# cristian-jfv/lattice-boltzmann-method

Hardware: AMD Instinct MI355X
Metric: MLUPS (million lattice updates/sec), D2Q9 BGK periodic box, f64 (higher is better)
Workload: dtype f64

## Files before the change

lattice-boltzmann-method_amd/csrc/capi_kbc.hip:

```cpp
#include "kbc.hpp"
#include "launch.hpp"

namespace lbm {

__global__ __launch_bounds__(256) void k_kbc_equilibrium(double* __restrict__ feq,
                                                         const double* __restrict__ m0,
                                                         const double* __restrict__ m1, long n,
                                                         int zero_u2) {
  for (long i = (long)blockIdx.x * 256 + threadIdx.x; i < n; i += (long)gridDim.x * 256) {
    const double ux = m1[i], uy = m1[n + i];
    const double ux2 = zero_u2 ? 0.0 : ux * ux, uy2 = zero_u2 ? 0.0 : uy * uy;
    double e[Q];
    KbcModel::feq_poly(e, ux, uy, ux2, uy2);
    const double r = m0[i];
#pragma unroll
    for (int q = 0; q < Q; ++q) feq[q * n + i] = e[q] * r;
  }
}

__global__ __launch_bounds__(256) void k_kbc_collide_given(double* __restrict__ out,
                                                           const double* __restrict__ f,
                                                           const double* __restrict__ m0,
                                                           const double* __restrict__ m1, long n,
                                                           KbcModel m) {
// ... 75 lines not shown
static int launch_stream_collide_sw_kbc(const char* fn, double* pn, const double* po,
                                        const lbm_geom* lg, const lbm_bc* lbc, const KbcFastModel& m,
                                        int depth, int row_begin, int row_end, hipStream_t st) {
  SwArgs a;
  int rc = sw_check_args(fn, pn, po, lg, lbc, depth, row_begin, row_end, sw_full_strips<KbcFastModel>::value, kSwKbc, &a);
  if (rc || !a.nrows) return rc;
  if (a.walls) {
    rc = depth == 2 ? sw_launch_walls<KbcFastModel, 2>(pn, po, a.g, m, a.bc, row_begin, row_end, st)
                    : sw_launch_walls<KbcFastModel, 3>(pn, po, a.g, m, a.bc, row_begin, row_end, st);
    if (rc) return rc;
    LBM_CHECK_LAUNCH();
    return LBM_OK;
  }
  auto launch = [&](auto D, auto LDSR) {
    constexpr int DV = decltype(D)::value;
    const SwPlan p = sw_plan(k_stream_collide_sw<KbcFastModel, DV, 2, true, false, false, LDSR()>, 128, a.nrows, a.strips, depth);
    LBM_KLAUNCH((k_stream_collide_sw<KbcFastModel, DV, 2, true, false, false, LDSR()>), dim3((p.n_waves + 1) / 2), dim3(128), 0, st, pn, po, a.g, m,
                row_begin, row_end, p.rpc, a.strips, p.n_waves, tuning("sw_xcd", 0));
  };
  with_flags([&](auto LDSR) {
    switch (depth) {
      case 2: launch(std::integral_constant<int, 2>{}, LDSR); break;
      case 3: launch(std::integral_constant<int, 3>{}, LDSR); break;
      default: launch(std::integral_constant<int, 4>{}, LDSR); break;
    }
  }, tuning("sw_ldsring", 1) != 0);
  LBM_CHECK_LAUNCH();
  return LBM_OK;
}

}
int lbm::kbc_stream_collide_x2_ref(double* pn, const double* po, const lbm_geom* lg, const lbm_bc* lbc,
                                   const lbm_kbc_params* prm, int row_begin, int row_end, hipStream_t st) {
// ... 126 lines not shown
```

lattice-boltzmann-method_amd/csrc/d2q9.hpp:

```cpp
#pragma once
#include <type_traits>
#include <hip/hip_runtime.h>

#include "../../include/lbm_hip.h"

namespace lbm {

constexpr int Q = 9;

#define LBM_W0 (4.0 / 9.0)
#define LBM_WS (1.0 / 9.0)
#define LBM_WD (1.0 / 36.0)

__device__ __forceinline__ constexpr double wq(int q) {
  return q == 0 ? LBM_W0 : (q < 5 ? LBM_WS : LBM_WD);
}
__host__ __device__ __forceinline__ constexpr int icx(int q) {
  return (q == 1 || q == 5 || q == 8) ? 1 : ((q == 3 || q == 6 || q == 7) ? -1 : 0);
}
__host__ __device__ __forceinline__ constexpr int icy(int q) {
  return (q == 2 || q == 5 || q == 6) ? 1 : ((q == 4 || q == 7 || q == 8) ? -1 : 0);
}
__host__ __device__ __forceinline__ constexpr int opp(int q) {
  return q == 0 ? 0 : (q == 1 ? 3 : (q == 2 ? 4 : (q == 3 ? 1 : (q == 4 ? 2 : (q == 5 ? 7 : (q == 6 ? 8 : (q == 7 ? 5 : 6)))))));
// ... 603 lines not shown
  (void)c_load;
}

#ifdef LBM_EXPERIMENTS
#include "experiments/sw_prefetch2.hpp"
#endif

__host__ __device__ constexpr int sw_strip_width(int D, bool full = false) {
  return full ? 64 - 2 * (D - 1) : (64 - 2 * (D - 1)) / 8 * 8;
}
template <class M, class = void>
struct sw_full_strips : std::false_type {};
template <class M>
struct sw_full_strips<M, std::void_t<decltype(M::kFullStrips)>> : std::bool_constant<M::kFullStrips> {};
__host__ __device__ constexpr int sw_waves_per_simd(int D) { return D <= 2 ? 4 : (D == 3 ? 3 : (D <= 5 ? 2 : 1)); }
template <class Model, int D, bool NT_STORE, bool HAS_BC, bool PF2, bool LDSR = false>
__device__ __forceinline__ void sw_wave_body(double* __restrict__ pn, const double* __restrict__ po, const Geom& g,
                                             const Model& m, int row_begin, int row_end, int rows_per_chunk, int strips,
                                             int wave, int lane, const Bc& bc, int strip0, int chunk_stride,
                                             double* lds = nullptr) {
  static_assert(!(LDSR && (HAS_BC || PF2)), "the LDS ring exists for the plain window only");
  constexpr int W = sw_strip_width(D, sw_full_strips<Model>::value);
  const int strip = strip0 + wave % strips, chunk = wave / strips;
  const int R0 = row_begin + chunk * (chunk_stride > 0 ? chunk_stride : rows_per_chunk);
  const int R1 = R0 + rows_per_chunk < row_end ? R0 + rows_per_chunk : row_end;
  int c = strip * W - (D - 1) + lane;
  const int c_raw = c;
  const bool lane_ok = lane >= D - 1 && lane < D - 1 + W && c < g.C;
  const bool walled_cols = HAS_BC && (bc_is_wall(bc.col_lo) || bc_is_wall(bc.col_hi));
  if (walled_cols) {
    c = c < 0 ? 0 : (c > g.C - 1 ? g.C - 1 : c);
  } else {
    c = c < 0 ? c + g.C : (c >= g.C ? c - g.C : c);
    c = c >= g.C ? c - g.C : c;
  }
  const int cols[3] = {walled_cols ? (c + 1 > g.C - 1 ? g.C - 1 : c + 1) : wrap_col(g, c + 1), c,
                       walled_cols ? (c - 1 < 0 ? 0 : c - 1) : wrap_col(g, c - 1)};
  const int rbase = R0 - (D - 1);
  const int n_iter = (R1 - R0) + 2 * (D - 1);
  double ring[D > 1 ? D - 1 : 1][3][Q];
// ... 44 lines not shown
  if constexpr (LDSR) {
    for (int k = lane; k < sw_lds_ring_doubles(D); k += 64) lds[k] = 1.0;
    __builtin_amdgcn_fence(__ATOMIC_RELEASE, "wavefront");
    __builtin_amdgcn_wave_barrier();
    __builtin_amdgcn_fence(__ATOMIC_ACQUIRE, "wavefront");
  }
  for (int i = 0; i < n_iter; i += 3) {
    sw_iteration<Model, D, 0, NT_STORE, HAS_BC, LDSR>(ring, cur, pn, po, g, m, i, rbase, R0, R1, c, cols, lane_ok, c, bc, c_bc, lds, lane);
    sw_iteration<Model, D, 1, NT_STORE, HAS_BC, LDSR>(ring, cur, pn, po, g, m, i + 1, rbase, R0, R1, c, cols, lane_ok, c, bc, c_bc, lds, lane);
    sw_iteration<Model, D, 2, NT_STORE, HAS_BC, LDSR>(ring, cur, pn, po, g, m, i + 2, rbase, R0, R1, c, cols, lane_ok, c, bc, c_bc, lds, lane);
  }
}

template <class Model, int D, int WAVES, bool NT_STORE, bool HAS_BC = false, bool PF2 = false, bool LDSR = false>
__global__ __launch_bounds__(64 * WAVES, (LDSR ? 2 : (WAVES == 4 ? sw_waves_per_simd(D) : 1))) void k_stream_collide_sw(
    double* __restrict__ pn, const double* __restrict__ po, Geom g, Model m, int row_begin,
    int row_end, int rows_per_chunk, int strips, int n_waves, int xcd_group, Bc bc = Bc{}, int strip0 = 0,
    int chunk_stride = 0) {
  int blk = blockIdx.x;
  if (xcd_group > 0) {
    const int x = blk % 8, mth = blk / 8, win = 8 * xcd_group;
    if ((mth / xcd_group + 1) * win <= (int)gridDim.x) blk = (mth / xcd_group) * win + x * xcd_group + mth % xcd_group;
  }
  const int wave = blk * WAVES + __builtin_amdgcn_readfirstlane(threadIdx.x >> 6), lane = threadIdx.x & 63;
  if (wave >= n_waves) return;
  if constexpr (LDSR) {
    __shared__ double lring[WAVES * sw_lds_ring_doubles(D)];
    sw_wave_body<Model, D, NT_STORE, HAS_BC, PF2, true>(pn, po, g, m, row_begin, row_end, rows_per_chunk, strips, wave, lane, bc, strip0, chunk_stride,
                                                        lring + (threadIdx.x >> 6) * sw_lds_ring_doubles(D));
  } else {
    sw_wave_body<Model, D, NT_STORE, HAS_BC, PF2>(pn, po, g, m, row_begin, row_end, rows_per_chunk, strips, wave, lane, bc, strip0, chunk_stride);
  }
}

struct SwPart {
  int r0, r1, s0, ns, rpc, wave0;
};
struct SwParts {
  SwPart p[5];
  int n_frame_waves, n_waves;
};
template <class Model, int D, bool NT_STORE>
__global__ __launch_bounds__(128, 1) void k_stream_collide_sw_walls(double* __restrict__ pn, const double* __restrict__ po,
                                                                    Geom g, Model m, Bc bc, SwParts parts) {
  const int wave = blockIdx.x * 2 + __builtin_amdgcn_readfirstlane(threadIdx.x >> 6), lane = threadIdx.x & 63;
  if (wave >= parts.n_waves) return;
  if (wave < parts.n_frame_waves) {
    int k = 0;
#pragma unroll
    for (int a = 1; a < 4; ++a)
      if (parts.p[a].ns > 0 && parts.p[a].r1 > parts.p[a].r0 && wave >= parts.p[a].wave0) k = a;
    const SwPart pt = parts.p[k];
    sw_wave_body<Model, D, NT_STORE, true, false>(pn, po, g, m, pt.r0, pt.r1, pt.rpc, pt.ns, wave - pt.wave0, lane, bc, pt.s0, 0);
  } else {
    const SwPart pt = parts.p[4];
    sw_wave_body<Model, D, NT_STORE, false, false>(pn, po, g, m, pt.r0, pt.r1, pt.rpc, pt.ns, wave - pt.wave0, lane, bc, pt.s0, 0);
  }
}

#ifdef LBM_EXPERIMENTS
#include "experiments/sw_paired_strips.hpp"
#endif
#ifdef LBM_EXPERIMENTS
#include "experiments/sw_two_columns.hpp"
#endif

template <class Model, bool WITH_MOMENTS>
__global__ __launch_bounds__(256) void k_edge_stream_collide(
    double* __restrict__ pn, const double* __restrict__ po, Geom g, Bc bc, Model m, int row_begin,
    int row_end, double* __restrict__ rho_out, double* __restrict__ u_out) {
  const int i = blockIdx.x * blockDim.x + threadIdx.x, n = row_end - row_begin;
// ... 52 lines not shown
```

lattice-boltzmann-method_amd/csrc/experiments/cg_launch.hpp:

```cpp
constexpr bool kCgExperiments = true;
constexpr int kCgNotMine = 1;

template <class Kernel>
static SwPlan cg_exp_chunks(Kernel* kernel, int block_threads, int nrows, int strips, int depth = 3, int rows_unfitted = 64) {
  return sw_plan(kernel, block_threads, nrows, strips, depth, 0, "cg_rows2", rows_unfitted);
}

template <int WAVES>
static int launch_cg_strip_t(const CgStepArgs& a, hipStream_t st) {
  int rpc = tuning("cg_rows", 16);
  const int nrows = a.row_end - a.row_begin;
  if (rpc > nrows) rpc = nrows;
  const int strips = (a.g.C + CG_SW - 1) / CG_SW, chunks = (nrows + rpc - 1) / rpc;
  const int n_waves = strips * chunks;
  const dim3 grid((n_waves + WAVES - 1) / WAVES);
  with_flags([&](auto PSI) { LBM_KLAUNCH((k_cg_strip<WAVES, PSI()>), grid, dim3(64 * WAVES), 0, st, a.pn_r, a.pn_b, a.in_r, a.in_b, a.g, a.bc, a.cf, a.rho_r, a.rho_b, a.u, a.psi, a.snu, a.mi, a.row_begin, a.row_end, rpc, strips, n_waves); }, a.psi != nullptr);
  LBM_CHECK_LAUNCH();
  return LBM_OK;
}

template <int TR, int TC, int WAVES>
static int cg_exp_one_launch(const CgStepArgs& a, const CgPlan& p, int part, int xs, hipStream_t st) {
  switch (a.g.P != a.g.C ? 0 : tuning("cg_strip", 0)) {
    case 0: break;
// ... 13 lines not shown
  with_flags([&](auto PSI) { LBM_KLAUNCH((k_cg_tile_mn<BR, BC, BT, BM, BP, PSI()>), dim3(p.n_btr * p.n_btc), dim3(BT), 0, st, a.pn_r, a.pn_b, a.in_r, a.in_b, a.g, a.cf, a.rho_r, a.rho_b, a.u, a.psi, a.snu, a.mi, ra, ca, p.n_btc, p.big_xcd); }, a.psi != nullptr);
}

static void cg_exp_walk_tile(const CgStepArgs& a, const CgPlan& p, int ra, int ca, hipStream_t st) {
  int rpc = tuning("cg_walk_rows", 128) / 16 * 16;
  if (rpc < 16) rpc = 16;
  const int rows_total = p.n_btr * 16, chunks = (rows_total + rpc - 1) / rpc;
  const int wx = tuning("cg_walk_tile_xcd", 2);
  with_flags([&](auto PSI) { LBM_KLAUNCH((k_cg_walk_tile<PSI()>), dim3(chunks * p.n_btc), dim3(512), 0, st, a.pn_r, a.pn_b, a.in_r, a.in_b, a.g, a.cf, a.rho_r, a.rho_b, a.u, a.psi, a.snu, a.mi, ra, ca, p.n_btc, rows_total, rpc, wx); }, a.psi != nullptr);
}

template <int WV>
static void cg_exp_strip2(const CgStepArgs& a, int ra, int rb, int ca, int cb, hipStream_t st) {
  const int strips = (cb - ca + CG_SW2 - 1) / CG_SW2;
  with_flags([&](auto PSI) {
    const SwPlan c = cg_exp_chunks(k_cg_strip2<WV, PSI()>, 64 * WV, rb - ra, strips);
    LBM_KLAUNCH((k_cg_strip2<WV, PSI()>), dim3((c.n_waves + WV - 1) / WV), dim3(64 * WV), 0, st, a.pn_r, a.pn_b, a.in_r, a.in_b, a.g, a.cf, a.rho_r, a.rho_b, a.u, a.psi, a.snu, a.mi, ra, rb, ca, cb, c.rpc, strips, c.n_waves);
  }, a.psi != nullptr);
}

template <int WV>
static void cg_exp_strip3(const CgStepArgs& a, int ra, int rb, int ca, int cb, hipStream_t st) {
  const int strips = (cb - ca + CG_SW2 - 1) / CG_SW2;
  const int xo = tuning("cg_strip_xcd", 0);
  with_flags([&](auto PSI) {
    const SwPlan c = cg_exp_chunks(k_cg_strip3<WV, PSI()>, 64 * WV, rb - ra, strips);
    const int nblk = (c.n_waves + WV - 1) / WV, grid = xo ? ((nblk + 7) / 8) * 8 : nblk;
    LBM_KLAUNCH((k_cg_strip3<WV, PSI()>), dim3(grid), dim3(64 * WV), 0, st, a.pn_r, a.pn_b, a.in_r, a.in_b, a.g, a.cf, a.rho_r, a.rho_b, a.u, a.psi, a.snu, a.mi, ra, rb, ca, cb, c.rpc, strips, c.n_waves, xo);
  }, a.psi != nullptr);
}

template <int WV>
static void cg_exp_strip4(const CgStepArgs& a, int ra, int rb, int ca, int cb, hipStream_t st) {
  constexpr int S = 64 * WV - 2 * CG_S4_EDGE;
  const int win0 = (ca - CG_S4_EDGE) / 16 * 16;
  const int bstrips = (cb - (win0 + CG_S4_EDGE) + S - 1) / S;
  with_flags([&](auto PSI) {
    const int rpc = cg_exp_chunks(k_cg_strip4<WV, PSI()>, 64 * WV, rb - ra, bstrips * WV).rpc;
    const int chunks = (rb - ra + rpc - 1) / rpc;
    LBM_KLAUNCH((k_cg_strip4<WV, PSI()>), dim3(bstrips * chunks), dim3(64 * WV), 0, st, a.pn_r, a.pn_b, a.in_r, a.in_b, a.g, a.cf, a.rho_r, a.rho_b, a.u, a.psi, a.snu, a.mi, ra, rb, ca, cb, rpc, bstrips, win0);
  }, a.psi != nullptr);
// ... 143 lines not shown
```

lattice-boltzmann-method_amd/csrc/launch.hpp:

```cpp
#pragma once
#include <map>
#include <mutex>
#include <utility>
#include "d2q9.hpp"
#include "internal.hpp"

namespace lbm {

inline int validate_geom_bc(const char* fn, const lbm_geom* g, const lbm_bc* bc, bool reads_neighbours = true) {
  LBM_REQUIRE(g, "%s: NULL geometry", fn);
  LBM_REQUIRE(g->R >= 1 && g->C >= 1, "%s: R=%d C=%d must be positive", fn, g->R, g->C);
  LBM_REQUIRE(g->ghost >= 0 && g->ghost <= 15, "%s: ghost=%d must be 0..15", fn, g->ghost);
  LBM_REQUIRE(g->row_pitch == 0 || (g->row_pitch >= g->C && g->row_pitch % 2 == 0), "%s: row_pitch=%d must be even and >= C=%d (0 = dense)",
              fn, g->row_pitch, g->C);
  LBM_REQUIRE(g->plane_stride == 0 || g->plane_stride >= (long long)(g->R + 2 * g->ghost) * (g->row_pitch > 0 ? g->row_pitch : g->C),
              "%s: plane_stride=%lld smaller than a plane", fn, g->plane_stride);
  if (bc) {
    auto row_ok = [](int m) {
      return m == LBM_EDGE_PERIODIC || m == LBM_EDGE_HALO || m == LBM_EDGE_BOUNCE_BACK ||
             m == LBM_EDGE_ABB_VELOCITY;
    };
    auto col_ok = [](int m) {
      return m == LBM_EDGE_PERIODIC || m == LBM_EDGE_BOUNCE_BACK || m == LBM_EDGE_SPECULAR ||
             m == LBM_EDGE_WRAP_NOSHIFT;
// ... 117 lines not shown
    with_flags([&](auto NS) {                                                                     \
      LBM_KLAUNCH((k_stream_collide_tb2<Model, TRV, BV, NS()>), dim3((unsigned)nblk), dim3(BV), 0, st, pn, po, g, m, \
                  row_begin, row_end, tiles_x, tiles_y, order);                                   \
    }, nt);                                                                                       \
  } else
  LBM_TB2(4, 256) LBM_TB2(6, 256) LBM_TB2(8, 256) LBM_TB2(8, 512) LBM_TB2(12, 256) LBM_TB2(12, 512)
  LBM_TB2(14, 512) LBM_TB2(16, 512) LBM_TB2(16, 1024) LBM_TB2(30, 1024) {
    set_error("%s: no two-step instantiation for tb_rows=%d tb_block=%d", fn, tr, block);
    return LBM_ERR_INVALID;
  }
#undef LBM_TB2
  LBM_CHECK_LAUNCH();
  return LBM_OK;
}

inline int sw_pick_rows(int nrows, int strips, int depth, long slots) {
  auto cost = [&](int rows) {
    const long waves = (long)strips * ((nrows + rows - 1) / rows);
    const long rounds = (waves + slots - 1) / slots;
    return (double)rounds * (rows + 2 * (depth - 1)) * (1.0 + 0.25 / ((double)rounds * (double)rounds));
  };
  int best = nrows < 64 ? nrows : 64;
  double best_cost = cost(best) * 0.95;
  for (int rows = 32; rows <= 256 && rows <= nrows; rows += 4) {
    const double c = cost(rows);
    if (c < best_cost) best = rows, best_cost = c;
  }
  return best;
}

inline long sw_wave_slots(const void* kernel, int block_threads) {
  static std::mutex mu;
  static std::map<std::pair<const void*, int>, long> cache;
  int dev = 0;
  if (hipGetDevice(&dev) != hipSuccess) {
    (void)hipGetLastError();
    return 0;
  }
  std::lock_guard<std::mutex> lk(mu);
  auto it = cache.find({kernel, dev});
  if (it != cache.end()) return it->second;
  int blocks_per_cu = 0, cus = 0;
  long slots = 0;
  if (hipOccupancyMaxActiveBlocksPerMultiprocessor(&blocks_per_cu, kernel, block_threads, 0) == hipSuccess &&
      hipDeviceGetAttribute(&cus, hipDeviceAttributeMultiprocessorCount, dev) == hipSuccess && blocks_per_cu > 0 && cus > 0)
    slots = (long)blocks_per_cu * (block_threads / 64) * cus;
  else
    (void)hipGetLastError();
  cache[{kernel, dev}] = slots;
  return slots;
}

struct SwPlan {
  int rpc, n_waves;
};
template <class Kernel>
SwPlan sw_plan(Kernel* kernel, int block_threads, int nrows, int strips, int depth, int rows_fixed = 0,
               const char* rows_key = "sw_rows", int rows_unfitted = 64) {
  int rpc = rows_fixed > 0 ? rows_fixed : tuning(rows_key, -1);
  if (rpc <= 0) {
    const long slots = sw_wave_slots((const void*)kernel, block_threads);
    rpc = slots > 0 ? sw_pick_rows(nrows, strips, depth, slots) : rows_unfitted;
  }
  if (rpc > nrows) rpc = nrows;
  return {rpc, strips * ((nrows + rpc - 1) / rpc)};
}

template <class Model, int DV, bool HAS_BC>
void sw_launch_part(double* pn, const double* po, const Geom& g, const Model& m, const Bc& bc, int r0,
                    int r1, int s0, int ns, int rows_fixed, hipStream_t st) {
  if (r0 >= r1 || ns <= 0) return;
  const SwPlan p = sw_plan(k_stream_collide_sw<Model, DV, 2, true, HAS_BC>, 128, r1 - r0, ns, DV, rows_fixed);
  LBM_KLAUNCH((k_stream_collide_sw<Model, DV, 2, true, HAS_BC>), dim3((p.n_waves + 1) / 2), dim3(128), 0, st, pn, po, g, m,
              r0, r1, p.rpc, ns, p.n_waves, 0, bc, s0);
}

struct SwSideStream : SideStream {
  int dev = -1;
};
inline SideStream* sw_side_stream() {
  static thread_local SwSideStream side[16];
  int dev = 0;
  if (hipGetDevice(&dev) != hipSuccess || dev < 0 || dev >= 16) return nullptr;
  SwSideStream& s = side[dev];
  if (s.dev != dev) {
    if (s.create()) {
      (void)hipGetLastError();
      return nullptr;
    }
// ... 13 lines not shown
  if (bc_is_wall(bc.row_hi)) rb = row_end < g.R - 16 ? row_end : g.R - 16;
  if (col_walls) {
    s0 = 1;
    s1 = (g.C - W - DV) / W + 1;
    if (s1 > strips) s1 = strips;
  }
  int split = tuning("sw_split", -1);
  if (split < 0) split = (row_begin == 0 && row_end == g.R && !g.ghost) ? 1 : 2;
  if (split == 0 || ra >= rb || s0 >= s1) {
    sw_launch_part<Model, DV, true>(pn, po, g, m, bc, row_begin, row_end, 0, strips, 0, st);
    return LBM_OK;
  }
  if (split == 2) {
    SwParts pp{};
    const int fr = 8;
    auto part = [&](int k, int r0, int r1, int s0f, int ns, int rpc, int& wave0) {
      if (r1 < r0) r1 = r0;
      if (ns < 0) ns = 0;
      if (rpc > r1 - r0) rpc = r1 - r0;
      pp.p[k] = SwPart{r0, r1, s0f, ns, rpc > 0 ? rpc : 1, wave0};
      if (r1 > r0 && ns > 0) wave0 += ns * ((r1 - r0 + pp.p[k].rpc - 1) / pp.p[k].rpc);
    };
    int w0 = 0;
    part(0, row_begin, row_end, 0, s0, fr, w0);
    part(1, row_begin, row_end, s1, strips - s1, fr, w0);
    part(2, row_begin, ra, s0, s1 - s0, fr, w0);
    part(3, rb, row_end, s0, s1 - s0, fr, w0);
    pp.n_frame_waves = w0;
    part(4, ra, rb, s0, s1 - s0, sw_plan(k_stream_collide_sw_walls<Model, DV, true>, 128, rb - ra, s1 - s0, DV).rpc, w0);
    pp.n_waves = w0;
    LBM_KLAUNCH((k_stream_collide_sw_walls<Model, DV, true>), dim3((pp.n_waves + 1) / 2), dim3(128), 0, st, pn, po, g, m, bc, pp);
    return LBM_OK;
  }
  SideStream* sd = sw_side_stream();
  if (sd && !sd->try_fork(st)) sd = nullptr;
  hipStream_t fs = sd ? sd->st : st;
  sw_launch_part<Model, DV, true>(pn, po, g, m, bc, row_begin, row_end, 0, s0, 8, fs);
  sw_launch_part<Model, DV, true>(pn, po, g, m, bc, row_begin, row_end, s1, strips - s1, 8, fs);
  sw_launch_part<Model, DV, true>(pn, po, g, m, bc, row_begin, ra, s0, s1 - s0, 8, fs);
  sw_launch_part<Model, DV, true>(pn, po, g, m, bc, rb, row_end, s0, s1 - s0, 8, fs);
  sw_launch_part<Model, DV, false>(pn, po, g, m, bc, ra, rb, s0, s1 - s0, 0, st);
  return sd ? sd->join(st) : LBM_OK;
}

struct SwLimits {
// ... 49 lines not shown
    const Bc b2 = make_bc(lbc);
    if (bc_needs_edge_pass(b2)) {
      int rc2 = launch_stream_collide_sw(fn, pn, po, lg, lbc, m, depth, row_begin, row_end, st, default_waves);
      if (rc2) return rc2;
      return launch_stream_collide_sw(fn, pn, po, lg, lbc, m, depth, second_begin, second_begin + (row_end - row_begin), st, default_waves);
    }
  }
  SwArgs a;
  int rc = sw_check_args(fn, pn, po, lg, lbc, depth, row_begin, row_end, sw_full_strips<Model>::value, kSwBgk, &a);
  if (rc || !a.nrows) return rc;
  const Geom& g = a.g;
  const Bc& bc = a.bc;
  const int nrows = a.nrows, strips = a.strips;
  const int nt = tuning("nt", 3) & 2, waves = tuning("sw_waves", default_waves);
  auto plan = [&](auto* kernel, int block_threads, int n_strips, int plan_depth) {
    return second_begin >= 0 ? SwPlan{nrows, 2 * n_strips} : sw_plan(kernel, block_threads, nrows, n_strips, plan_depth);
  };
  const int chunk_stride = second_begin >= 0 ? second_begin - row_begin : 0;
  const int row_end_k = second_begin >= 0 ? second_begin + nrows : row_end;
  if (a.walls) {
#define LBM_SWBC(DV)                                                                              \
  if (depth == DV) {                                                                              \
    rc = sw_launch_walls<Model, DV>(pn, po, g, m, bc, row_begin, row_end, st);                    \
    if (rc) return rc;                                                                            \
  } else
    LBM_SWBC(2) LBM_SWBC(3) LBM_SWBC(4) LBM_SWBC(5) {
      set_error("%s: no wall-carrying sliding-window instantiation for depth=%d", fn, depth);
      return LBM_ERR_INVALID;
    }
#undef LBM_SWBC
    LBM_CHECK_LAUNCH();
    return LBM_OK;
  }
  bool launched = false;
#ifdef LBM_EXPERIMENTS
  if constexpr (std::is_same<Model, BgkFastModel>::value || std::is_same<Model, BgkModelT<0, 0>>::value) {
    const int pw = tuning("sw_pair", 0);
    if ((pw == 2 || pw == 4) && depth == 5 && nt && g.C >= 256) {
      const int GW = swp_group_width(5, pw), groups = (g.C + GW - 1) / GW;
      auto launch = [&](auto pw_c) {
        constexpr int PW = decltype(pw_c)::value;
        const SwPlan p = plan(k_stream_collide_swp<Model, 5, PW, true>, 64 * PW, groups * PW, 7);
        const int total = p.n_waves / PW;
        LBM_KLAUNCH((k_stream_collide_swp<Model, 5, PW, true>), dim3(total), dim3(64 * PW), 0, st, pn, po, g, m, row_begin, row_end_k, p.rpc, groups, total, chunk_stride);
      };
      if (pw == 4) launch(std::integral_constant<int, 4>{}); else launch(std::integral_constant<int, 2>{});
      launched = true;
    }
  }
  if constexpr (std::is_same<Model, BgkFastModel>::value) {
    if (!launched && tuning("sw_cols2", 0) && (depth == 5 || depth == 6) && nt && g.C % 2 == 0 && g.P % 2 == 0 && g.plane % 2 == 0 &&
        ((uintptr_t)pn % 16) == 0 && ((uintptr_t)po % 16) == 0) {
      const int W2 = sw2_strip_width(depth), strips2 = (g.C + W2 - 1) / W2;
      auto launch = [&](auto depth_c) {
        constexpr int DV = decltype(depth_c)::value;
        const SwPlan p = plan(k_stream_collide_sw2<Model, DV, true>, 128, strips2, depth);
        LBM_KLAUNCH((k_stream_collide_sw2<Model, DV, true>), dim3((p.n_waves + 1) / 2), dim3(128), 0, st, pn, po, g, m, row_begin, row_end_k, p.rpc, strips2, p.n_waves, chunk_stride);
      };
      if (depth == 6) launch(std::integral_constant<int, 6>{}); else launch(std::integral_constant<int, 5>{});
      launched = true;
    }
  }
  if constexpr (std::is_same<Model, BgkFastModel>::value) {
    if (!launched && tuning("sw_pf2", 0) && depth == 5 && waves == 2 && nt) {
      const SwPlan p = plan(k_stream_collide_sw<Model, 5, 2, true, false, true>, 128, strips, depth);
      LBM_KLAUNCH((k_stream_collide_sw<Model, 5, 2, true, false, true>), dim3((p.n_waves + 1) / 2), dim3(128), 0, st, pn, po, g, m,
                  row_begin, row_end_k, p.rpc, strips, p.n_waves, tuning("sw_xcd", 0), Bc{}, 0, chunk_stride);
      launched = true;
    }
  }
#endif
  if (!launched) {
#define LBM_SW(DV, WV)                                                                            \
  if (depth == DV && waves == WV) {                                                               \
    const SwPlan p = plan(k_stream_collide_sw<Model, DV, WV, true>, 64 * WV, strips, depth);      \
    with_flags([&](auto NS) {                                                                     \
      LBM_KLAUNCH((k_stream_collide_sw<Model, DV, WV, NS()>), dim3((p.n_waves + WV - 1) / WV), dim3(64 * WV), 0, st, pn, po, \
                  g, m, row_begin, row_end_k, p.rpc, strips, p.n_waves, tuning("sw_xcd", 0), Bc{}, 0, chunk_stride); \
    }, nt);                                                                                       \
  } else
  LBM_SW(2, 4) LBM_SW(3, 4) LBM_SW(4, 4) LBM_SW(5, 4) LBM_SW(6, 4)
  LBM_SW(2, 1) LBM_SW(3, 1) LBM_SW(4, 1) LBM_SW(2, 2) LBM_SW(3, 2) LBM_SW(4, 2) LBM_SW(5, 2) LBM_SW(6, 2) {
    set_error("%s: no sliding-window instantiation for depth=%d sw_waves=%d", fn, depth, waves);
    return LBM_ERR_INVALID;
  }
  }
#undef LBM_SW
  LBM_CHECK_LAUNCH();
  return LBM_OK;
}

template <class Model>
int launch_collide_only(const char* fn, double* p, const double* f, const lbm_geom* lg,
// ... 16 lines not shown
```

lattice-boltzmann-method_amd/pylbm/__init__.py:

```python
import ctypes as ct
import os
import re

import numpy as np

_HERE = os.path.dirname(os.path.abspath(__file__))
PKG_DIR = os.path.dirname(_HERE)
REPO = os.path.dirname(PKG_DIR)
LIB_PATH = os.environ.get("LBM_HIP_LIB", os.path.join(PKG_DIR, "lib", "liblbm_hip.so"))
HEADER = os.path.join(REPO, "include", "lbm_hip.h")

EDGE_PERIODIC, EDGE_HALO, EDGE_BOUNCE_BACK, EDGE_SPECULAR, EDGE_ABB_VELOCITY, EDGE_WRAP_NOSHIFT = range(6)
HALO_TWO_PHASE = -3
MODEL_BGK, MODEL_KBC = 0, 1
FORM_DEFAULT, FORM_REFERENCE_ORDER, FORM_REASSOCIATED = 0, 1, 2
RING_DEFAULT, RING_RCCL, RING_IPC = -1, 0, 1
CG_PART_FRAME, CG_PART_INNER = 1, 2
ADE_PART_FRAME, ADE_PART_INNER = 1, 2
ADE_SCALAR_NO_FLUX, ADE_SCALAR_FIXED = 0, 1
ADE_FACE_ROW_POS, ADE_FACE_ROW_NEG, ADE_FACE_COL_POS, ADE_FACE_COL_NEG = 0x91, 0x64, 0x32, 0xC8

ADE_OPEN_BOUNCE_BACK, ADE_OPEN_SPECULAR_ROW, ADE_OPEN_SPECULAR_COL, ADE_OPEN_ABB, ADE_OPEN_ABB_EXTRAPOLATED = 1, 2, 3, 4, 5

DIAG_NQ = 17
# ... 270 lines not shown
        assert table.ndim == 2 and table.shape[0] == DIAG_NQ, table.shape
        out = np.empty(DIAG_NQ)
        self.__getattr__("diag_fold_host")(_hptr(out), _hptr(table), table.shape[1], int(row_begin),
                                           int(table.shape[1] if row_end is None else row_end))
        return out

    def wallx_fold_host(self, table, row_begin=0, row_end=None):
        table = np.ascontiguousarray(table, dtype=np.float64)
        assert table.ndim == 2 and table.shape[0] == WALLX_NQ, table.shape
        out = np.empty(WALLX_NQ)
        self.__getattr__("ade_wallx_fold_host")(_hptr(out), _hptr(table), table.shape[1], int(row_begin),
                                                int(table.shape[1] if row_end is None else row_end))
        return out

    def reset_tuning(self):
        for k in (b"variant", b"nt", b"grid_cap", b"block", b"rows", b"xcd_swizzle", b"tb_rows", b"tb_block", b"tb_order", b"sw_rows", b"sw_waves", b"solver_depth", b"cg_fused", b"cg_tile", b"cg_xcd", b"kbc_fast", b"kbc_depth", b"bgk_fast", b"cg_strip", b"cg_rows", b"cg_split", b"sw_split", b"solver_depth_walls", b"ibm_depth", b"ibm_gate", b"bgk_fast_delta", b"pressure_depth", b"halo_grid", b"cg_strip2", b"cg_rows2", b"sw_pair", b"sw_pf2", b"cg_strip_xcd", b"cg_merge", b"cg_frame_beside", b"ring_period", b"ibm_step_opt", b"ibm_step_split", b"ibm_step_chain", b"ibm_box", b"ibm_box_overlap", b"bg_priority", b"ibm_chain_kernel", b"ibm_chain_wgs", b"ibm_box_sole", b"sw_ldsring", b"ring_ipc_timeout_ms", b"cg_big", b"cg_big_xcd", b"ring_ipc_force_cached", b"ring_ipc_cached_ok", b"row_pad", b"cg_walk_rows", b"cg_walk_tile_xcd", b"sw_cols2"):
            self.set_tuning(k, -1)


def _ptr(t):
    if t is None:
        return ct.cast(None, _dp)
    if isinstance(t, int):
        return ct.cast(t, _dp)
    assert t.stride(-1) == 1 and str(t.dtype) == "torch.float64", (t.dtype, t.stride())
    return ct.cast(t.data_ptr(), _dp)


def _hptr(a):
    assert a.dtype == np.float64 and a.flags["C_CONTIGUOUS"]
    return a.ctypes.data_as(_dp)
# ... 299 lines not shown
```

Before: 170,600.

## Plan graded-height row chunks for sliding-window kernel to balance wave makespan

Replaces the single uniform rows-per-chunk split in the sliding-window stream-collide kernels with a per-launch table of variable chunk heights. A host-side planner simulates wave scheduling on the available slots, tries tall-then-shrinking chunk sequences, and falls back to uniform chunks when those simulate faster. The goal is to cut tail imbalance in the last scheduling round, where some slots sit idle. In exchange, each kernel takes a larger by-value argument struct and does a table lookup per wave, and the host pays a cached planning search.

```diff
diff --git a/lattice-boltzmann-method_amd/csrc/capi_kbc.hip b/lattice-boltzmann-method_amd/csrc/capi_kbc.hip
--- a/lattice-boltzmann-method_amd/csrc/capi_kbc.hip
+++ b/lattice-boltzmann-method_amd/csrc/capi_kbc.hip
@@ -113,9 +113,9 @@
   }
   auto launch = [&](auto D, auto LDSR) {
     constexpr int DV = decltype(D)::value;
-    const SwPlan p = sw_plan(k_stream_collide_sw<KbcFastModel, DV, 2, true, false, false, LDSR()>, 128, a.nrows, a.strips, depth);
+    const SwPlan p = sw_plan(k_stream_collide_sw<KbcFastModel, DV, 2, true, false, false, LDSR()>, 128, row_begin, a.nrows, a.strips, depth);
     LBM_KLAUNCH((k_stream_collide_sw<KbcFastModel, DV, 2, true, false, false, LDSR()>), dim3((p.n_waves + 1) / 2), dim3(128), 0, st, pn, po, a.g, m,
-                row_begin, row_end, p.rpc, a.strips, p.n_waves, tuning("sw_xcd", 0));
+                row_end, p.chunks, a.strips, p.n_waves, tuning("sw_xcd", 0));
   };
   with_flags([&](auto LDSR) {
     switch (depth) {
diff --git a/lattice-boltzmann-method_amd/csrc/d2q9.hpp b/lattice-boltzmann-method_amd/csrc/d2q9.hpp
--- a/lattice-boltzmann-method_amd/csrc/d2q9.hpp
+++ b/lattice-boltzmann-method_amd/csrc/d2q9.hpp
@@ -641,16 +641,26 @@
 template <class M>
 struct sw_full_strips<M, std::void_t<decltype(M::kFullStrips)>> : std::bool_constant<M::kFullStrips> {};
 __host__ __device__ constexpr int sw_waves_per_simd(int D) { return D <= 2 ? 4 : (D == 3 ? 3 : (D <= 5 ? 2 : 1)); }
+constexpr int kSwTableChunks = 96;
+struct SwChunk {
+  int r0, rows;
+};
+struct SwChunks {
+  int n;
+  SwChunk c[kSwTableChunks];
+};
+__device__ __forceinline__ void sw_chunk_rows(const SwChunk* __restrict__ tab, int n, int chunk, int row_end, int& R0, int& R1) {
+  const int k = chunk < n - 1 ? chunk : n - 1;
+  const SwChunk e = tab[k];
+  R0 = e.r0 + (chunk - k) * e.rows;
+  R1 = R0 + e.rows < row_end ? R0 + e.rows : row_end;
+}
 template <class Model, int D, bool NT_STORE, bool HAS_BC, bool PF2, bool LDSR = false>
 __device__ __forceinline__ void sw_wave_body(double* __restrict__ pn, const double* __restrict__ po, const Geom& g,
-                                             const Model& m, int row_begin, int row_end, int rows_per_chunk, int strips,
-                                             int wave, int lane, const Bc& bc, int strip0, int chunk_stride,
+                                             const Model& m, int R0, int R1, int strip, int lane, const Bc& bc,
                                              double* lds = nullptr) {
   static_assert(!(LDSR && (HAS_BC || PF2)), "the LDS ring exists for the plain window only");
   constexpr int W = sw_strip_width(D, sw_full_strips<Model>::value);
-  const int strip = strip0 + wave % strips, chunk = wave / strips;
-  const int R0 = row_begin + chunk * (chunk_stride > 0 ? chunk_stride : rows_per_chunk);
-  const int R1 = R0 + rows_per_chunk < row_end ? R0 + rows_per_chunk : row_end;
   int c = strip * W - (D - 1) + lane;
   const int c_raw = c;
   const bool lane_ok = lane >= D - 1 && lane < D - 1 + W && c < g.C;
@@ -725,9 +735,8 @@
 
 template <class Model, int D, int WAVES, bool NT_STORE, bool HAS_BC = false, bool PF2 = false, bool LDSR = false>
 __global__ __launch_bounds__(64 * WAVES, (LDSR ? 2 : (WAVES == 4 ? sw_waves_per_simd(D) : 1))) void k_stream_collide_sw(
-    double* __restrict__ pn, const double* __restrict__ po, Geom g, Model m, int row_begin,
-    int row_end, int rows_per_chunk, int strips, int n_waves, int xcd_group, Bc bc = Bc{}, int strip0 = 0,
-    int chunk_stride = 0) {
+    double* __restrict__ pn, const double* __restrict__ po, Geom g, Model m, int row_end, SwChunks chunks,
+    int strips, int n_waves, int xcd_group, Bc bc = Bc{}, int strip0 = 0) {
   int blk = blockIdx.x;
   if (xcd_group > 0) {
     const int x = blk % 8, mth = blk / 8, win = 8 * xcd_group;
@@ -735,21 +744,24 @@
   }
   const int wave = blk * WAVES + __builtin_amdgcn_readfirstlane(threadIdx.x >> 6), lane = threadIdx.x & 63;
   if (wave >= n_waves) return;
+  int R0, R1;
+  sw_chunk_rows(chunks.c, chunks.n, wave / strips, row_end, R0, R1);
+  const int strip = strip0 + wave % strips;
   if constexpr (LDSR) {
     __shared__ double lring[WAVES * sw_lds_ring_doubles(D)];
-    sw_wave_body<Model, D, NT_STORE, HAS_BC, PF2, true>(pn, po, g, m, row_begin, row_end, rows_per_chunk, strips, wave, lane, bc, strip0, chunk_stride,
-                                                        lring + (threadIdx.x >> 6) * sw_lds_ring_doubles(D));
+    sw_wave_body<Model, D, NT_STORE, HAS_BC, PF2, true>(pn, po, g, m, R0, R1, strip, lane, bc, lring + (threadIdx.x >> 6) * sw_lds_ring_doubles(D));
   } else {
-    sw_wave_body<Model, D, NT_STORE, HAS_BC, PF2>(pn, po, g, m, row_begin, row_end, rows_per_chunk, strips, wave, lane, bc, strip0, chunk_stride);
+    sw_wave_body<Model, D, NT_STORE, HAS_BC, PF2>(pn, po, g, m, R0, R1, strip, lane, bc);
   }
 }
 
 struct SwPart {
-  int r0, r1, s0, ns, rpc, wave0;
+  int r0, r1, s0, ns, wave0, tab0, ntab;
 };
 struct SwParts {
   SwPart p[5];
   int n_frame_waves, n_waves;
+  SwChunk tab[kSwTableChunks + 4];
 };
 template <class Model, int D, bool NT_STORE>
 __global__ __launch_bounds__(128, 1) void k_stream_collide_sw_walls(double* __restrict__ pn, const double* __restrict__ po,
@@ -762,10 +774,14 @@
     for (int a = 1; a < 4; ++a)
       if (parts.p[a].ns > 0 && parts.p[a].r1 > parts.p[a].r0 && wave >= parts.p[a].wave0) k = a;
     const SwPart pt = parts.p[k];
-    sw_wave_body<Model, D, NT_STORE, true, false>(pn, po, g, m, pt.r0, pt.r1, pt.rpc, pt.ns, wave - pt.wave0, lane, bc, pt.s0, 0);
+    int R0, R1;
+    sw_chunk_rows(parts.tab + pt.tab0, pt.ntab, (wave - pt.wave0) / pt.ns, pt.r1, R0, R1);
+    sw_wave_body<Model, D, NT_STORE, true, false>(pn, po, g, m, R0, R1, pt.s0 + (wave - pt.wave0) % pt.ns, lane, bc);
   } else {
     const SwPart pt = parts.p[4];
-    sw_wave_body<Model, D, NT_STORE, false, false>(pn, po, g, m, pt.r0, pt.r1, pt.rpc, pt.ns, wave - pt.wave0, lane, bc, pt.s0, 0);
+    int R0, R1;
+    sw_chunk_rows(parts.tab + pt.tab0, pt.ntab, (wave - pt.wave0) / pt.ns, pt.r1, R0, R1);
+    sw_wave_body<Model, D, NT_STORE, false, false>(pn, po, g, m, R0, R1, pt.s0 + (wave - pt.wave0) % pt.ns, lane, bc);
   }
 }
 
diff --git a/lattice-boltzmann-method_amd/csrc/experiments/cg_launch.hpp b/lattice-boltzmann-method_amd/csrc/experiments/cg_launch.hpp
--- a/lattice-boltzmann-method_amd/csrc/experiments/cg_launch.hpp
+++ b/lattice-boltzmann-method_amd/csrc/experiments/cg_launch.hpp
@@ -2,8 +2,8 @@
 constexpr int kCgNotMine = 1;
 
 template <class Kernel>
-static SwPlan cg_exp_chunks(Kernel* kernel, int block_threads, int nrows, int strips, int depth = 3, int rows_unfitted = 64) {
-  return sw_plan(kernel, block_threads, nrows, strips, depth, 0, "cg_rows2", rows_unfitted);
+static SwUniform cg_exp_chunks(Kernel* kernel, int block_threads, int nrows, int strips, int depth = 3, int rows_unfitted = 64) {
+  return sw_plan_uniform(kernel, block_threads, nrows, strips, depth, 0, "cg_rows2", rows_unfitted);
 }
 
 template <int WAVES>
@@ -51,7 +51,7 @@
 static void cg_exp_strip2(const CgStepArgs& a, int ra, int rb, int ca, int cb, hipStream_t st) {
   const int strips = (cb - ca + CG_SW2 - 1) / CG_SW2;
   with_flags([&](auto PSI) {
-    const SwPlan c = cg_exp_chunks(k_cg_strip2<WV, PSI()>, 64 * WV, rb - ra, strips);
+    const SwUniform c = cg_exp_chunks(k_cg_strip2<WV, PSI()>, 64 * WV, rb - ra, strips);
     LBM_KLAUNCH((k_cg_strip2<WV, PSI()>), dim3((c.n_waves + WV - 1) / WV), dim3(64 * WV), 0, st, a.pn_r, a.pn_b, a.in_r, a.in_b, a.g, a.cf, a.rho_r, a.rho_b, a.u, a.psi, a.snu, a.mi, ra, rb, ca, cb, c.rpc, strips, c.n_waves);
   }, a.psi != nullptr);
 }
@@ -61,7 +61,7 @@
   const int strips = (cb - ca + CG_SW2 - 1) / CG_SW2;
   const int xo = tuning("cg_strip_xcd", 0);
   with_flags([&](auto PSI) {
-    const SwPlan c = cg_exp_chunks(k_cg_strip3<WV, PSI()>, 64 * WV, rb - ra, strips);
+    const SwUniform c = cg_exp_chunks(k_cg_strip3<WV, PSI()>, 64 * WV, rb - ra, strips);
     const int nblk = (c.n_waves + WV - 1) / WV, grid = xo ? ((nblk + 7) / 8) * 8 : nblk;
     LBM_KLAUNCH((k_cg_strip3<WV, PSI()>), dim3(grid), dim3(64 * WV), 0, st, a.pn_r, a.pn_b, a.in_r, a.in_b, a.g, a.cf, a.rho_r, a.rho_b, a.u, a.psi, a.snu, a.mi, ra, rb, ca, cb, c.rpc, strips, c.n_waves, xo);
   }, a.psi != nullptr);
diff --git a/lattice-boltzmann-method_amd/csrc/launch.hpp b/lattice-boltzmann-method_amd/csrc/launch.hpp
--- a/lattice-boltzmann-method_amd/csrc/launch.hpp
+++ b/lattice-boltzmann-method_amd/csrc/launch.hpp
@@ -1,9 +1,12 @@
 #pragma once
 #include <map>
 #include <mutex>
+#include <tuple>
 #include <utility>
+#include <vector>
 #include "d2q9.hpp"
 #include "internal.hpp"
+#include "sw_plan.hpp"
 
 namespace lbm {
 
@@ -155,21 +158,6 @@
   return LBM_OK;
 }
 
-inline int sw_pick_rows(int nrows, int strips, int depth, long slots) {
-  auto cost = [&](int rows) {
-    const long waves = (long)strips * ((nrows + rows - 1) / rows);
-    const long rounds = (waves + slots - 1) / slots;
-    return (double)rounds * (rows + 2 * (depth - 1)) * (1.0 + 0.25 / ((double)rounds * (double)rounds));
-  };
-  int best = nrows < 64 ? nrows : 64;
-  double best_cost = cost(best) * 0.95;
-  for (int rows = 32; rows <= 256 && rows <= nrows; rows += 4) {
-    const double c = cost(rows);
-    if (c < best_cost) best = rows, best_cost = c;
-  }
-  return best;
-}
-
 inline long sw_wave_slots(const void* kernel, int block_threads) {
   static std::mutex mu;
   static std::map<std::pair<const void*, int>, long> cache;
@@ -192,12 +180,12 @@
   return slots;
 }
 
-struct SwPlan {
+struct SwUniform {
   int rpc, n_waves;
 };
 template <class Kernel>
-SwPlan sw_plan(Kernel* kernel, int block_threads, int nrows, int strips, int depth, int rows_fixed = 0,
-               const char* rows_key = "sw_rows", int rows_unfitted = 64) {
+SwUniform sw_plan_uniform(Kernel* kernel, int block_threads, int nrows, int strips, int depth, int rows_fixed = 0,
+                          const char* rows_key = "sw_rows", int rows_unfitted = 64) {
   int rpc = rows_fixed > 0 ? rows_fixed : tuning(rows_key, -1);
   if (rpc <= 0) {
     const long slots = sw_wave_slots((const void*)kernel, block_threads);
@@ -207,13 +195,67 @@
   return {rpc, strips * ((nrows + rpc - 1) / rpc)};
 }
 
+inline std::vector<int> sw_graded_chunks(int nrows, int strips, int depth, long slots, int tall_cap) {
+  static std::mutex mu;
+  static std::map<std::tuple<int, int, int, long, int>, std::vector<int>> cache;
+  std::lock_guard<std::mutex> lk(mu);
+  auto it = cache.find({nrows, strips, depth, slots, tall_cap});
+  if (it == cache.end()) {
+    std::vector<int> h = sw_plan_chunks(nrows, strips, depth, slots, tall_cap);
+    if (sw_uniform_wins(h, nrows, strips, depth, slots)) h.clear();
+    it = cache.emplace(std::make_tuple(nrows, strips, depth, slots, tall_cap), h).first;
+  }
+  return it->second;
+}
+
+constexpr int kSwTallCap = 192;
+struct SwPlan {
+  int n_waves;
+  SwChunks chunks;
+};
+inline SwPlan sw_plan_of_heights(const std::vector<int>& h, int row_begin, int strips) {
+  SwPlan p{};
+  int r = row_begin;
+  for (int k = 0; k < (int)h.size() && k < kSwTableChunks; ++k) p.chunks.c[p.chunks.n++] = SwChunk{r, h[k]}, r += h[k];
+  p.n_waves = strips * p.chunks.n;
+  return p;
+}
+template <class Kernel>
+SwPlan sw_plan(Kernel* kernel, int block_threads, int row_begin, int nrows, int strips, int depth, int rows_fixed = 0) {
+  static_assert(kSwTableChunks >= kSwMaxChunks, "a planned launch must fit the kernel's table");
+  int rpc = rows_fixed > 0 ? rows_fixed : tuning("sw_rows", -1);
+  if (rpc <= 0 && tuning("sw_test_h0", 0) > 0) {
+    static const char* const keys[8] = {"sw_test_h0", "sw_test_h1", "sw_test_h2", "sw_test_h3", "sw_test_h4", "sw_test_h5", "sw_test_h6", "sw_test_h7"};
+    std::vector<int> h;
+    for (int rem = nrows, i = 0; rem > 0; i = (i + 1) % 8) {
+      int hk = tuning(keys[i], 0);
+      if (hk <= 0) hk = tuning(keys[i = 0], 1);
+      if (hk > rem || (int)h.size() == kSwTableChunks - 1) hk = rem;
+      h.push_back(hk), rem -= hk;
+    }
+    return sw_plan_of_heights(h, row_begin, strips);
+  }
+  if (rpc <= 0 && tuning("sw_plan", 1) != 0) {
+    const long slots = sw_wave_slots((const void*)kernel, block_threads);
+    const int cap = tuning("sw_tall_cap", kSwTallCap);
+    const std::vector<int> h = sw_graded_chunks(nrows, strips, depth, slots, cap > 0 ? cap : kSwTallCap);
+    if (!h.empty()) return sw_plan_of_heights(h, row_begin, strips);
+  }
+  const SwUniform u = sw_plan_uniform(kernel, block_threads, nrows, strips, depth, rpc > 0 ? rpc : 0);
+  SwPlan p{};
+  p.n_waves = u.n_waves;
+  p.chunks.n = 1;
+  p.chunks.c[0] = SwChunk{row_begin, u.rpc};
+  return p;
+}
+
 template <class Model, int DV, bool HAS_BC>
 void sw_launch_part(double* pn, const double* po, const Geom& g, const Model& m, const Bc& bc, int r0,
                     int r1, int s0, int ns, int rows_fixed, hipStream_t st) {
   if (r0 >= r1 || ns <= 0) return;
-  const SwPlan p = sw_plan(k_stream_collide_sw<Model, DV, 2, true, HAS_BC>, 128, r1 - r0, ns, DV, rows_fixed);
+  const SwPlan p = sw_plan(k_stream_collide_sw<Model, DV, 2, true, HAS_BC>, 128, r0, r1 - r0, ns, DV, rows_fixed);
   LBM_KLAUNCH((k_stream_collide_sw<Model, DV, 2, true, HAS_BC>), dim3((p.n_waves + 1) / 2), dim3(128), 0, st, pn, po, g, m,
-              r0, r1, p.rpc, ns, p.n_waves, 0, bc, s0);
+              r1, p.chunks, ns, p.n_waves, 0, bc, s0);
 }
 
 struct SwSideStream : SideStream {
@@ -257,21 +299,24 @@
   if (split == 2) {
     SwParts pp{};
     const int fr = 8;
-    auto part = [&](int k, int r0, int r1, int s0f, int ns, int rpc, int& wave0) {
+    int w0 = 0;
+    auto frame = [&](int k, int r0, int r1, int s0f, int ns) {
       if (r1 < r0) r1 = r0;
       if (ns < 0) ns = 0;
-      if (rpc > r1 - r0) rpc = r1 - r0;
-      pp.p[k] = SwPart{r0, r1, s0f, ns, rpc > 0 ? rpc : 1, wave0};
-      if (r1 > r0 && ns > 0) wave0 += ns * ((r1 - r0 + pp.p[k].rpc - 1) / pp.p[k].rpc);
+      const int rpc = r1 - r0 < fr ? (r1 > r0 ? r1 - r0 : 1) : fr;
+      pp.p[k] = SwPart{r0, r1, s0f, ns, w0, k, 1};
+      pp.tab[k] = SwChunk{r0, rpc};
+      if (r1 > r0 && ns > 0) w0 += ns * ((r1 - r0 + rpc - 1) / rpc);
     };
-    int w0 = 0;
-    part(0, row_begin, row_end, 0, s0, fr, w0);
-    part(1, row_begin, row_end, s1, strips - s1, fr, w0);
-    part(2, row_begin, ra, s0, s1 - s0, fr, w0);
-    part(3, rb, row_end, s0, s1 - s0, fr, w0);
+    frame(0, row_begin, row_end, 0, s0);
+    frame(1, row_begin, row_end, s1, strips - s1);
+    frame(2, row_begin, ra, s0, s1 - s0);
+    frame(3, rb, row_end, s0, s1 - s0);
     pp.n_frame_waves = w0;
-    part(4, ra, rb, s0, s1 - s0, sw_plan(k_stream_collide_sw_walls<Model, DV, true>, 128, rb - ra, s1 - s0, DV).rpc, w0);
-    pp.n_waves = w0;
+    const SwPlan in = sw_plan(k_stream_collide_sw_walls<Model, DV, true>, 128, ra, rb - ra, s1 - s0, DV);
+    pp.p[4] = SwPart{ra, rb, s0, s1 - s0, w0, 4, in.chunks.n};
+    for (int k = 0; k < in.chunks.n; ++k) pp.tab[4 + k] = in.chunks.c[k];
+    pp.n_waves = w0 + in.n_waves;
     LBM_KLAUNCH((k_stream_collide_sw_walls<Model, DV, true>), dim3((pp.n_waves + 1) / 2), dim3(128), 0, st, pn, po, g, m, bc, pp);
     return LBM_OK;
   }
@@ -351,10 +396,21 @@
   const int nrows = a.nrows, strips = a.strips;
   const int nt = tuning("nt", 3) & 2, waves = tuning("sw_waves", default_waves);
   auto plan = [&](auto* kernel, int block_threads, int n_strips, int plan_depth) {
-    return second_begin >= 0 ? SwPlan{nrows, 2 * n_strips} : sw_plan(kernel, block_threads, nrows, n_strips, plan_depth);
+    if (second_begin < 0) return sw_plan(kernel, block_threads, row_begin, nrows, n_strips, plan_depth);
+    SwPlan p{};
+    p.n_waves = 2 * n_strips;
+    p.chunks.n = 2;
+    p.chunks.c[0] = SwChunk{row_begin, nrows};
+    p.chunks.c[1] = SwChunk{second_begin, nrows};
+    return p;
+  };
+  const int row_end_k = second_begin >= 0 ? second_begin + nrows : row_end;
+#ifdef LBM_EXPERIMENTS
+  auto plan_uniform = [&](auto* kernel, int block_threads, int n_strips, int plan_depth) {
+    return second_begin >= 0 ? SwUniform{nrows, 2 * n_strips} : sw_plan_uniform(kernel, block_threads, nrows, n_strips, plan_depth);
   };
   const int chunk_stride = second_begin >= 0 ? second_begin - row_begin : 0;
-  const int row_end_k = second_begin >= 0 ? second_begin + nrows : row_end;
+#endif
   if (a.walls) {
 #define LBM_SWBC(DV)                                                                              \
   if (depth == DV) {                                                                              \
@@ -377,7 +433,7 @@
       const int GW = swp_group_width(5, pw), groups = (g.C + GW - 1) / GW;
       auto launch = [&](auto pw_c) {
         constexpr int PW = decltype(pw_c)::value;
-        const SwPlan p = plan(k_stream_collide_swp<Model, 5, PW, true>, 64 * PW, groups * PW, 7);
+        const SwUniform p = plan_uniform(k_stream_collide_swp<Model, 5, PW, true>, 64 * PW, groups * PW, 7);
         const int total = p.n_waves / PW;
         LBM_KLAUNCH((k_stream_collide_swp<Model, 5, PW, true>), dim3(total), dim3(64 * PW), 0, st, pn, po, g, m, row_begin, row_end_k, p.rpc, groups, total, chunk_stride);
       };
@@ -391,7 +447,7 @@
       const int W2 = sw2_strip_width(depth), strips2 = (g.C + W2 - 1) / W2;
       auto launch = [&](auto depth_c) {
         constexpr int DV = decltype(depth_c)::value;
-        const SwPlan p = plan(k_stream_collide_sw2<Model, DV, true>, 128, strips2, depth);
+        const SwUniform p = plan_uniform(k_stream_collide_sw2<Model, DV, true>, 128, strips2, depth);
         LBM_KLAUNCH((k_stream_collide_sw2<Model, DV, true>), dim3((p.n_waves + 1) / 2), dim3(128), 0, st, pn, po, g, m, row_begin, row_end_k, p.rpc, strips2, p.n_waves, chunk_stride);
       };
       if (depth == 6) launch(std::integral_constant<int, 6>{}); else launch(std::integral_constant<int, 5>{});
@@ -402,7 +458,7 @@
     if (!launched && tuning("sw_pf2", 0) && depth == 5 && waves == 2 && nt) {
       const SwPlan p = plan(k_stream_collide_sw<Model, 5, 2, true, false, true>, 128, strips, depth);
       LBM_KLAUNCH((k_stream_collide_sw<Model, 5, 2, true, false, true>), dim3((p.n_waves + 1) / 2), dim3(128), 0, st, pn, po, g, m,
-                  row_begin, row_end_k, p.rpc, strips, p.n_waves, tuning("sw_xcd", 0), Bc{}, 0, chunk_stride);
+                  row_end_k, p.chunks, strips, p.n_waves, tuning("sw_xcd", 0));
       launched = true;
     }
   }
@@ -413,7 +469,7 @@
     const SwPlan p = plan(k_stream_collide_sw<Model, DV, WV, true>, 64 * WV, strips, depth);      \
     with_flags([&](auto NS) {                                                                     \
       LBM_KLAUNCH((k_stream_collide_sw<Model, DV, WV, NS()>), dim3((p.n_waves + WV - 1) / WV), dim3(64 * WV), 0, st, pn, po, \
-                  g, m, row_begin, row_end_k, p.rpc, strips, p.n_waves, tuning("sw_xcd", 0), Bc{}, 0, chunk_stride); \
+                  g, m, row_end_k, p.chunks, strips, p.n_waves, tuning("sw_xcd", 0));                               \
     }, nt);                                                                                       \
   } else
   LBM_SW(2, 4) LBM_SW(3, 4) LBM_SW(4, 4) LBM_SW(5, 4) LBM_SW(6, 4)
diff --git a/lattice-boltzmann-method_amd/csrc/sw_plan.hpp b/lattice-boltzmann-method_amd/csrc/sw_plan.hpp
--- /dev/null
+++ b/lattice-boltzmann-method_amd/csrc/sw_plan.hpp
@@ -0,0 +1,123 @@
+#pragma once
+#include <algorithm>
+#include <functional>
+#include <queue>
+#include <utility>
+#include <vector>
+
+namespace lbm {
+
+constexpr int kSwMaxChunks = 96;
+constexpr int kSwShortest = 32;
+
+inline int sw_pick_rows(int nrows, int strips, int depth, long slots) {
+  auto cost = [&](int rows) {
+    const long waves = (long)strips * ((nrows + rows - 1) / rows);
+    const long rounds = (waves + slots - 1) / slots;
+    return (double)rounds * (rows + 2 * (depth - 1)) * (1.0 + 0.25 / ((double)rounds * (double)rounds));
+  };
+  int best = nrows < 64 ? nrows : 64;
+  double best_cost = cost(best) * 0.95;
+  for (int rows = 32; rows <= 256 && rows <= nrows; rows += 4) {
+    const double c = cost(rows);
+    if (c < best_cost) best = rows, best_cost = c;
+  }
+  return best;
+}
+
+inline std::vector<int> sw_uniform_chunks(int nrows, int rows) {
+  std::vector<int> h;
+  if (rows < 1) rows = 1;
+  for (int r = 0; r < nrows; r += rows) h.push_back(nrows - r < rows ? nrows - r : rows);
+  return h;
+}
+
+using SwSlotHeap = std::priority_queue<std::pair<long, long>, std::vector<std::pair<long, long>>, std::greater<std::pair<long, long>>>;
+inline long sw_makespan_from(SwSlotHeap& q, long end, const int* h, int n, int strips, int depth) {
+  for (int i = 0; i < n;) {
+    int j = i;
+    while (j < n && h[j] == h[i]) ++j;
+    long waves = (long)strips * (j - i);
+    const long d = h[i] + 2 * (depth - 1);
+    while (waves > 0) {
+      const std::pair<long, long> e = q.top();
+      q.pop();
+      const long k = e.second < waves ? e.second : waves;
+      q.push({e.first + d, k});
+      if (e.second > k) q.push({e.first, e.second - k});
+      if (e.first + d > end) end = e.first + d;
+      waves -= k;
+    }
+    i = j;
+  }
+  return end;
+}
+inline long sw_makespan(const std::vector<int>& h, int strips, int depth, long slots) {
+  SwSlotHeap q;
+  q.push({0, slots > 0 ? slots : 1});
+  return sw_makespan_from(q, 0, h.data(), (int)h.size(), strips, depth);
+}
+
+inline std::vector<int> sw_plan_chunks(int nrows, int strips, int depth, long slots, int tall_cap) {
+  if (nrows <= 0) return {};
+  const int h_floor = (nrows + kSwMaxChunks - 1) / kSwMaxChunks;
+  if (slots <= 0) return sw_uniform_chunks(nrows, h_floor > 64 ? h_floor : 64);
+  if (nrows < 2 || strips < 1) return {nrows};
+  int cap = tall_cap < h_floor ? h_floor : tall_cap;
+  if (cap > nrows) cap = nrows;
+  std::vector<int> best, cand;
+  long best_t = -1;
+  auto offer = [&](const std::vector<int>& h, long t) {
+    if (best_t < 0 || t < best_t || (t == best_t && h.size() < best.size())) best = h, best_t = t;
+  };
+  for (int k = 1; k <= kSwMaxChunks && k <= nrows; ++k) {
+    const int rows = (nrows + k - 1) / k;
+    if (rows > cap || (rows < kSwShortest && k > 1)) continue;
+    cand = sw_uniform_chunks(nrows, rows);
+    offer(cand, sw_makespan(cand, strips, depth, slots));
+  }
+  const int picked = sw_pick_rows(nrows, strips, depth, slots);
+  if ((nrows + picked - 1) / picked <= kSwMaxChunks) {
+    cand = sw_uniform_chunks(nrows, picked);
+    offer(cand, sw_makespan(cand, strips, depth, slots));
+  }
+  static const double kRatio[] = {0.5, 0.65, 0.8, 0.9};
+  static const int kMin[] = {8, 16, 32, 64};
+  int last_H = 0;
+  for (int step = 16; step >= 1; --step) {
+    const int H = cap * step / 16;
+    if (H < kSwShortest || H == last_H) continue;
+    last_H = H;
+    for (int n_tall = 1; n_tall < kSwMaxChunks && (long)n_tall * H < nrows; ++n_tall) {
+      SwSlotHeap q0;
+      q0.push({0, slots});
+      const std::vector<int> tall(n_tall, H);
+      const long t0 = sw_makespan_from(q0, 0, tall.data(), n_tall, strips, depth);
+      if (best_t >= 0 && t0 >= best_t) break;
+      for (double ratio : kRatio)
+        for (int h_min : kMin) {
+          if (h_min >= H) continue;
+          cand = tall;
+          int rem = nrows - n_tall * H, h = H;
+          while (rem > 0 && (int)cand.size() < kSwMaxChunks) {
+            h = std::max({1, h_min, (int)(h * ratio)});
+            if (h > rem) h = rem;
+            cand.push_back(h);
+            rem -= h;
+          }
+          if (rem > 0) continue;
+          SwSlotHeap q = q0;
+          offer(cand, sw_makespan_from(q, t0, cand.data() + n_tall, (int)cand.size() - n_tall, strips, depth));
+        }
+    }
+  }
+  return best;
+}
+
+inline bool sw_uniform_wins(const std::vector<int>& planned, int nrows, int strips, int depth, long slots) {
+  if (slots <= 0 || nrows <= 0) return false;
+  return sw_makespan(sw_uniform_chunks(nrows, sw_pick_rows(nrows, strips, depth, slots)), strips, depth, slots) <
+         sw_makespan(planned, strips, depth, slots);
+}
+
+}
diff --git a/lattice-boltzmann-method_amd/drivers/sw_plan_dump.cpp b/lattice-boltzmann-method_amd/drivers/sw_plan_dump.cpp
--- /dev/null
+++ b/lattice-boltzmann-method_amd/drivers/sw_plan_dump.cpp
@@ -0,0 +1,28 @@
+#include <cstdio>
+
+#include "../csrc/sw_plan.hpp"
+
+int main() {
+  char line[256];
+  while (std::fgets(line, sizeof line, stdin)) {
+    int rows, cols, depth, cap = 192, strips = 0;
+    long slots;
+    const int n = std::sscanf(line, "%d %d %d %ld %d %d", &rows, &cols, &depth, &slots, &cap, &strips);
+    if (n <= 0) continue;
+    if (n < 4 || rows < 1 || cols < 1 || depth < 2 || depth > 8 || slots < 0 || cap < 1 || strips < 0) {
+      std::printf("{\"error\": \"bad case\"}\n");
+      return 2;
+    }
+    const int W = (64 - 2 * (depth - 1)) / 8 * 8;
+    if (strips == 0) strips = (cols + W - 1) / W;
+    const std::vector<int> h = lbm::sw_plan_chunks(rows, strips, depth, slots, cap);
+    const int urows = slots > 0 ? lbm::sw_pick_rows(rows, strips, depth, slots) : 64;
+    std::printf("{\"strips\": %d, \"heights\": [", strips);
+    for (size_t i = 0; i < h.size(); ++i) std::printf("%s%d", i ? ", " : "", h[i]);
+    std::printf("], \"makespan\": %ld, \"uniform_rows\": %d, \"uniform_makespan\": %ld, \"ideal\": %.1f, \"uniform_wins\": %d}\n",
+                lbm::sw_makespan(h, strips, depth, slots), urows < rows ? urows : rows,
+                lbm::sw_makespan(lbm::sw_uniform_chunks(rows, urows), strips, depth, slots),
+                slots > 0 ? (double)strips * rows / (double)slots : 0.0, (int)lbm::sw_uniform_wins(h, rows, strips, depth, slots));
+  }
+  return 0;
+}
diff --git a/lattice-boltzmann-method_amd/pylbm/__init__.py b/lattice-boltzmann-method_amd/pylbm/__init__.py
--- a/lattice-boltzmann-method_amd/pylbm/__init__.py
+++ b/lattice-boltzmann-method_amd/pylbm/__init__.py
@@ -308,7 +308,7 @@
         return out
 
     def reset_tuning(self):
-        for k in (b"variant", b"nt", b"grid_cap", b"block", b"rows", b"xcd_swizzle", b"tb_rows", b"tb_block", b"tb_order", b"sw_rows", b"sw_waves", b"solver_depth", b"cg_fused", b"cg_tile", b"cg_xcd", b"kbc_fast", b"kbc_depth", b"bgk_fast", b"cg_strip", b"cg_rows", b"cg_split", b"sw_split", b"solver_depth_walls", b"ibm_depth", b"ibm_gate", b"bgk_fast_delta", b"pressure_depth", b"halo_grid", b"cg_strip2", b"cg_rows2", b"sw_pair", b"sw_pf2", b"cg_strip_xcd", b"cg_merge", b"cg_frame_beside", b"ring_period", b"ibm_step_opt", b"ibm_step_split", b"ibm_step_chain", b"ibm_box", b"ibm_box_overlap", b"bg_priority", b"ibm_chain_kernel", b"ibm_chain_wgs", b"ibm_box_sole", b"sw_ldsring", b"ring_ipc_timeout_ms", b"cg_big", b"cg_big_xcd", b"ring_ipc_force_cached", b"ring_ipc_cached_ok", b"row_pad", b"cg_walk_rows", b"cg_walk_tile_xcd", b"sw_cols2"):
+        for k in (b"variant", b"nt", b"grid_cap", b"block", b"rows", b"xcd_swizzle", b"tb_rows", b"tb_block", b"tb_order", b"sw_rows", b"sw_waves", b"solver_depth", b"cg_fused", b"cg_tile", b"cg_xcd", b"kbc_fast", b"kbc_depth", b"bgk_fast", b"cg_strip", b"cg_rows", b"cg_split", b"sw_split", b"solver_depth_walls", b"ibm_depth", b"ibm_gate", b"bgk_fast_delta", b"pressure_depth", b"halo_grid", b"cg_strip2", b"cg_rows2", b"sw_pair", b"sw_pf2", b"cg_strip_xcd", b"cg_merge", b"cg_frame_beside", b"ring_period", b"ibm_step_opt", b"ibm_step_split", b"ibm_step_chain", b"ibm_box", b"ibm_box_overlap", b"bg_priority", b"ibm_chain_kernel", b"ibm_chain_wgs", b"ibm_box_sole", b"sw_ldsring", b"ring_ipc_timeout_ms", b"cg_big", b"cg_big_xcd", b"ring_ipc_force_cached", b"ring_ipc_cached_ok", b"row_pad", b"cg_walk_rows", b"cg_walk_tile_xcd", b"sw_cols2", b"sw_plan", b"sw_tall_cap") + tuple(b"sw_test_h%d" % i for i in range(8)):
             self.set_tuning(k, -1)
 
 
```

Result: no change. 171,100, median of 3 (+0.3%).
